# RatInABox-Lab/RatInABox

Hardware: AMD Instinct MI355X
Metric: agent-steps/sec (whole node) at 4096 agents x 1024 PlaceCells (higher is better)
Workload: dtype f32 rates / f64 motion

## Files before the change

ratinabox_amd/Neurons.py:

```python
import copy
import warnings

import numpy as np
import torch

from . import _lib, utils
from ._history import DeviceHistory, HistoryView

_Tensor = torch.Tensor

_L = _lib
LOG2E = 1.4426950408889634


def _pad4(n):
    return (int(n) + 3) // 4 * 4


class Neurons:
    default_params = {
        "n": 10,
        "name": "Neurons",
        "color": None,
        "noise_std": 0,
# ... 731 lines not shown
                self._window_stats = dict(share=self.BVC_WINDOW_SHARE, cells_need=float(keep.mean()))
                if not keep.all():
                    band = np.minimum(keep.sum(axis=1) // 24, 7)
                    order = np.lexsort((np.mod(mu_t, 2 * np.pi), band))
                    cells, vm, inv = cells[:, order], vm[order], inv[order]
                    keep = keep[order]
                    win = np.zeros(((n + 3) // 4, 2), dtype=np.int32)
                    for g in range(len(win)):
                        u = keep[np.minimum(np.arange(4 * g, 4 * g + 4), n - 1)].any(axis=0)
                        gap_len, gap_start, run = 0, 0, 0
                        for k in range(2 * K):
                            run = run + 1 if not u[k % K] else 0
                            if min(run, K) > gap_len:
                                gap_len, gap_start = min(run, K), (k - min(run, K) + 1) % K
                        first = (gap_start + gap_len) % K
                        k0 = first // 4 * 4
                        length = min(K, (first - k0 + (K - gap_len) + 3) // 4 * 4)
                        win[g] = (0, K) if length >= K else (k0, length)
                    rows_t = torch.from_numpy(order.astype(np.int32)).to(self._device)
                    win_t = torch.from_numpy(win).to(self._device)
                    self._window_stats["issued"] = float(win[:, 1].sum() * 4 / (len(win) * 4 * K))
            f32 = lambda x: torch.from_numpy(np.ascontiguousarray(x, dtype=np.float32)).to(self._device)
            s_w = walls[:, 1, :] - walls[:, 0, :]
            with np.errstate(divide="ignore"):
                rden = 1.0 / (dirs[:, None, 0] * (-s_w[None, :, 1]) + dirs[:, None, 1] * s_w[None, :, 0])
            f64 = lambda x: torch.from_numpy(np.ascontiguousarray(x, dtype=np.float64)).to(self._device)
            dirs_dev = dirs
            if os.environ.get("RIAB_EXP_NO_RAY_PAIRS"):
                dirs_dev = dirs.copy()
                dirs_dev[2, 0] += 1e-9
            return (f64(dirs_dev), f64(rden), f32(cells), f32(vm), f32(inv), rows_t, win_t)

        import os
        use_windows = os.environ.get("RIAB_NO_BVC_WINDOWS") is None
        walls = np.asarray(self.Agent.Environment.walls, dtype=np.float64).reshape(-1, 2, 2)
        dirs_t, rden_t, cells_t, vm_t, inv_t, rows_t, win_t = self._tables(
            (mu_d, sg_d, mu_t, sg_t, ang, dirs, norm, ego, walls, use_windows), build)
        if io is None:
            d = dict(kind=_L.POP_KINDS["bvc"], table=cells_t, test_dirs=dirs_t, ray_rden=rden_t, K=K, vm_table=vm_t,
                     inv_norm=inv_t, egocentric=1 if ego else 0)
            if rows_t is not None:
                d.update(cell_rows=rows_t, windows=win_t)
            return d
        env, _w = self.Agent.Environment.device_tables(self._device)
        rc = _L.lib.riab_boundary_vector_cells_windowed(env, io, _L.ptr(dirs_t), _L.ptr(rden_t), K, _L.ptr(cells_t),
                                                        _L.ptr(vm_t), _L.ptr(inv_t), n, 1 if ego else 0, None,
                                                        _L.ptr(rows_t), _L.ptr(win_t), stream)
        _L.check(rc, "riab_boundary_vector_cells")

    def _plan_scratch(self, pop):
        tiles, Kp = (self._Bp + 63) // 64, (int(pop.K) + 3) // 4 * 4
        if getattr(self, "_bvc_xch", None) is None or tuple(self._bvc_xch.shape) != (tiles, Kp, 64):
            self._bvc_xch = torch.empty((tiles, Kp, 64), dtype=torch.float32, device=self._device)
            self._bvc_xch_count = torch.zeros(tiles, dtype=torch.int32, device=self._device)
        else:
            self._bvc_xch_count.zero_()
        pop.bvc_xch, pop.bvc_xch_count = self._bvc_xch.data_ptr(), self._bvc_xch_count.data_ptr()

    def _state_op(self, d):
        from . import ops
        f = self._call(None, None)
        walls, env, periodic = self._env_op_args()
        ego = bool(f["egocentric"])
        return torch.ops.riab.boundary_vector_cells(d[0:2], d[2:4] if ego else None, walls, env, periodic, f["test_dirs"],
                                                    f["ray_rden"], f["table"], f["vm_table"], f["inv_norm"], ego,
                                                    f.get("cell_rows"), f.get("windows"), float(self.min_fr),
                                                    float(self.max_fr))


class FieldOfViewBVCs(BoundaryVectorCells):

    default_params = {
        "distance_range": [0.02, 0.4],
        "angle_range": [0, 75],
        "spatial_resolution": 0.02,
        "cell_arrangement": "diverging_manifold",
        "beta": 5,
        "color": [0.3, 0.3, 0.3, 1],
    }

    def __init__(self, Agent, params={}):
        self.params = copy.deepcopy(__class__.default_params)
        self.params.update(params)
        self.params["reference_frame"] = "egocentric"
        assert self.params["cell_arrangement"] is not None, "cell_arrangement must be set for FoV Neurons"
        self._warn_if_n_changes = "n" in params and params["n"] is not None
        super().__init__(Agent, self.params)


class ObjectVectorCells(VectorCells):

    default_params = {
        "n": 10,
        "name": "ObjectVectorCell",
        "walls_occlude": True,
        "object_tuning_type": "random",
    }

    def __init__(self, Agent, params={}):
        self.Agent = Agent
        self.params = copy.deepcopy(__class__.default_params)
        self.params.update(params)
        if not hasattr(self, "_warn_if_n_changes"):
            self._warn_if_n_changes = "n" in params and params["n"] is not None
        super().__init__(Agent, self.params)
        self.object_locations = self.Agent.Environment.objects["objects"]
        if len(self.object_locations) == 0:
            raise RuntimeError(f"Cannot initialize {self.params['name']}, as there are no objects in the environment.")
        self.tuning_types = None
        self.set_tuning_types(self.object_tuning_type)
# ... 585 lines not shown
```

ratinabox_amd/csrc/riab_bvc.hip:

```cpp
#include <type_traits>
#include "riab_device.h"
#include "riab_handover.h"
#include "riab_launch.h"

#ifndef RIAB_BVC_XCH_KB
#define RIAB_BVC_XCH_KB 1
#endif
namespace riab {

typedef float v4f __attribute__((ext_vector_type(4)));
typedef float v2f __attribute__((ext_vector_type(2)));

struct BvcArgs {
  const float* pos_x;
  const float* pos_y;
  const float* hd_x;
  const float* hd_y;
  int64_t pos_ld;
  int64_t P;
  int64_t B;
  float* rates;
  uint8_t* spikes;
  const float* u_in;
  float dt, fr_scale, fr_min;
  uint32_t k0, k1, step0, tag;
  int64_t agent_id0;
  int n, K, Kp, n_walls;
  const double* walls;
  const double* test_dirs;
  const double* ray_rden;
  const float* cells;
  const float* vm;
  const float* inv_norm;
  float* ray_out;
  const int* rows;
  const int* win;
  double e0, e1, e2, e3;
  int rect_room;
  float* xch;
  uint32_t* xch_count;
  uint32_t xch_target;
};

typedef const __attribute__((address_space(4))) double* const_f64_ptr;

template <int J>
__device__ __forceinline__ uint32_t quad_word(const u32x4& blk, int qi) {
  const uint32_t wx = (uint32_t)__builtin_amdgcn_mov_dpp((int)blk.x, J * 0x55, 0xF, 0xF, true);
  const uint32_t wy = (uint32_t)__builtin_amdgcn_mov_dpp((int)blk.y, J * 0x55, 0xF, 0xF, true);
  const uint32_t wz = (uint32_t)__builtin_amdgcn_mov_dpp((int)blk.z, J * 0x55, 0xF, 0xF, true);
  const uint32_t ww = (uint32_t)__builtin_amdgcn_mov_dpp((int)blk.w, J * 0x55, 0xF, 0xF, true);
  return qi == 0 ? wx : (qi == 1 ? wy : (qi == 2 ? wz : ww));
}

template <bool EGO>
__global__ __launch_bounds__(512) void bvc_kernel(const BvcArgs a) {
  extern __shared__ __align__(16) unsigned char smem[];
  float* s_d = reinterpret_cast<float*>(smem);
  const int tid = threadIdx.x, lane = tid & 63;
  const int wave = __builtin_amdgcn_readfirstlane(tid >> 6);
  const int nw = a.n_walls, K = a.K;
  const const_f64_ptr walls = (const_f64_ptr)(const void*)a.walls;
  const const_f64_ptr dirs = (const_f64_ptr)(const void*)a.test_dirs;
  const const_f64_ptr rden = (const_f64_ptr)(const void*)a.ray_rden;

  const int tile = (int)blockIdx.x, part = (int)blockIdx.y, nparts = (int)gridDim.y;
  const int64_t p = (int64_t)tile * 64 + lane;
  const bool live = p < a.P;
  const int64_t pc = live ? p : 0;
  const int64_t t = pc / a.B;
  const int64_t b = pc - t * a.B;
  const float pxf = a.pos_x[t * a.pos_ld + b], pyf = a.pos_y[t * a.pos_ld + b];
  const double px = pxf, py = pyf;

  bool box4 = false;
  if (a.rect_room && nw >= 4) {
    bool ok = true;
    int nh = 0, nv = 0;
    const double tol = 1e-9 * ((a.e1 - a.e0) + (a.e3 - a.e2));
    for (int w = 0; w < 4; ++w) {
      const double ax = walls[4 * w], ay = walls[4 * w + 1], bx = walls[4 * w + 2], by = walls[4 * w + 3];
      if (ay == by && ax != bx) {
        ++nh;
        ok = ok && (ay == a.e2 || ay == a.e3) && fmin(ax, bx) <= a.e0 + tol && fmax(ax, bx) >= a.e1 - tol;
      } else if (ax == bx && ay != by) {
        ++nv;
        ok = ok && (ax == a.e0 || ax == a.e1) && fmin(ay, by) <= a.e2 + tol && fmax(ay, by) >= a.e3 - tol;
      } else {
        ok = false;
      }
    }
    ok = ok && nh == 2 && nv == 2;
    const bool inside = px > a.e0 && px < a.e1 && py > a.e2 && py < a.e3;
    box4 = ok && __builtin_amdgcn_ballot_w64(live && !inside) == 0;
  }
  const int w_full = box4 ? 4 : 0;
  auto cast_rays = [&](auto KB_, const int vw, const int nvw, const bool publish) {
  constexpr int KB = decltype(KB_)::value;
  float* const xrow = publish ? a.xch + (int64_t)tile * a.Kp * 64 + lane : nullptr;
  auto put = [&](int k, float d) {
    s_d[k * 64 + lane] = d;
    if (publish) st_agent(xrow + k * 64, d);
  };
  auto stands_on_wall = [&](const double ux, const double uy, const int k) -> bool {
    for (int w = 0; w < nw; ++w) {
      const double ax = walls[4 * w], ay = walls[4 * w + 1];
      const double sx = walls[4 * w + 2] - ax, sy = walls[4 * w + 3] - ay;
      const double d0x = ax - px, d0y = ay - py;
      const double rd = rden[k * nw + w];
      const double la = (d0x * (-sy) + d0y * sx) * rd;
      const double lb = ((-d0x) * (-uy) + (-d0y) * ux) * (-rd);
      if (la == 0.0 && !(lb < 0.0) && !(lb > 1.0)) return true;
    }
    return false;
  };
  auto cast_single = [&](int count, int off) {
    for (int t0 = vw; t0 < count; t0 += nvw * KB) {
      double ux[KB], uy[KB], best[KB], fallback[KB];
      int kk[KB];
#pragma unroll
      for (int i = 0; i < KB; ++i) {
        const int t = min(t0 + nvw * i, count - 1);
        kk[i] = t == 0 ? 0 : t + off;
        ux[i] = dirs[2 * kk[i]];
        uy[i] = dirs[2 * kk[i] + 1];
        best[i] = INFINITY;
        fallback[i] = 0.0;
      }
      for (int w = 0; w < w_full; ++w) {
        const double ax = walls[4 * w], ay = walls[4 * w + 1];
        const double sx = walls[4 * w + 2] - ax, sy = walls[4 * w + 3] - ay;
        const double d0x = ax - px, d0y = ay - py;
        const double num_a = d0x * (-sy) + d0y * sx;
#pragma unroll
        for (int i = 0; i < KB; ++i) {
          const double la = num_a * rden[kk[i] * nw + w];
          if (la > 0.0 && la < best[i]) best[i] = la;
          if (w == 0) fallback[i] = la;
        }
      }
      for (int w = w_full; w < nw; ++w) {
        const double ax = walls[4 * w], ay = walls[4 * w + 1];
        const double sx = walls[4 * w + 2] - ax, sy = walls[4 * w + 3] - ay;
        const double d0x = ax - px, d0y = ay - py;
        const double num_a = d0x * (-sy) + d0y * sx;
#pragma unroll
        for (int i = 0; i < KB; ++i) {
          const double rd = rden[kk[i] * nw + w];
          const double la = num_a * rd;
          const double lb = ((-d0x) * (-uy[i]) + (-d0y) * ux[i]) * (-rd);
          const bool valid = (la > 0.0) && !(lb < 0.0) && !(lb > 1.0);
          if (valid && la < best[i]) best[i] = la;
          if (w == 0) fallback[i] = la;
        }
      }
#pragma unroll
      for (int i = 0; i < KB; ++i) {
        if (t0 + nvw * i < count) {
          const int k = kk[i];
          const bool hit = best[i] < INFINITY;
          const float d = (float)(hit ? best[i] : (stands_on_wall(ux[i], uy[i], k) ? 0.0 : fallback[i]));
          put(k, d);
          if (a.ray_out && live && (publish || part == 0)) a.ray_out[(t * K + k) * a.B + b] = d;
        }
      }
    }
  };
  const int m = K >> 1, np = K - 1 - m;
  bool paired = false;
  if ((K & 1) == 0 && np >= 8) {
    bool ok = true;
    for (int jq = 1 + lane; jq <= np; jq += 64) {
      const double e0 = a.test_dirs[2 * jq] + a.test_dirs[2 * (jq + m)];
      const double e1 = a.test_dirs[2 * jq + 1] + a.test_dirs[2 * (jq + m) + 1];
      ok = ok && fabs(e0) <= 1e-12 && fabs(e1) <= 1e-12;
    }
    paired = __builtin_amdgcn_ballot_w64(!ok) == 0;
  }
  if (paired) {
    for (int q0 = vw; q0 < np; q0 += nvw * KB) {
      double ux[KB], uy[KB], bpos[KB], bneg[KB], fallback[KB];
      int jj[KB];
#pragma unroll
      for (int i = 0; i < KB; ++i) {
        jj[i] = 1 + min(q0 + nvw * i, np - 1);
        ux[i] = dirs[2 * jj[i]];
        uy[i] = dirs[2 * jj[i] + 1];
        bpos[i] = INFINITY;
        bneg[i] = INFINITY;
        fallback[i] = 0.0;
      }
      for (int w = 0; w < w_full; ++w) {
        const double ax = walls[4 * w], ay = walls[4 * w + 1];
        const double sx = walls[4 * w + 2] - ax, sy = walls[4 * w + 3] - ay;
        const double d0x = ax - px, d0y = ay - py;
        const double num_a = d0x * (-sy) + d0y * sx;
#pragma unroll
        for (int i = 0; i < KB; ++i) {
          const double la = num_a * rden[jj[i] * nw + w];
          const double nla = -la;
          if (la > 0.0 && la < bpos[i]) bpos[i] = la;
          if (nla > 0.0 && nla < bneg[i]) bneg[i] = nla;
          if (w == 0) fallback[i] = la;
        }
      }
      for (int w = w_full; w < nw; ++w) {
        const double ax = walls[4 * w], ay = walls[4 * w + 1];
        const double sx = walls[4 * w + 2] - ax, sy = walls[4 * w + 3] - ay;
        const double d0x = ax - px, d0y = ay - py;
        const double num_a = d0x * (-sy) + d0y * sx;
#pragma unroll
        for (int i = 0; i < KB; ++i) {
          const double rd = rden[jj[i] * nw + w];
          const double la = num_a * rd;
          const double lb = ((-d0x) * (-uy[i]) + (-d0y) * ux[i]) * (-rd);
          const bool on_wall = !(lb < 0.0) && !(lb > 1.0);
          const double nla = -la;
          if (on_wall && la > 0.0 && la < bpos[i]) bpos[i] = la;
          if (on_wall && nla > 0.0 && nla < bneg[i]) bneg[i] = nla;
          if (w == 0) fallback[i] = la;
        }
      }
#pragma unroll
      for (int i = 0; i < KB; ++i) {
        if (q0 + nvw * i < np) {
          const int k = jj[i];
          const bool hit_p = bpos[i] < INFINITY, hit_n = bneg[i] < INFINITY;
          const bool on = !(hit_p && hit_n) && stands_on_wall(ux[i], uy[i], k);
          const float dp = (float)(hit_p ? bpos[i] : (on ? 0.0 : fallback[i]));
          const float dn = (float)(hit_n ? bneg[i] : (on ? 0.0 : -fallback[i]));
          put(k, dp);
          put(k + m, dn);
          if (a.ray_out && live && (publish || part == 0)) {
            a.ray_out[(t * K + k) * a.B + b] = dp;
            a.ray_out[(t * K + k + m) * a.B + b] = dn;
          }
        }
      }
    }
    cast_single(1 + (m - np), np);
  } else {
    cast_single(K, 0);
  }
  };
  const bool exchange = a.xch != nullptr && nparts > 1;
  if (!exchange) {
    cast_rays(std::integral_constant<int, 4>{}, wave, 8, false);
  } else {
    cast_rays(std::integral_constant<int, RIAB_BVC_XCH_KB>{}, wave + 8 * part, 8 * nparts, true);
    drain_stores();
    __syncthreads();
    __shared__ int s_all_here;
    if (tid == 0) {
      uint32_t* const cnt = a.xch_count + tile;
      fetch_add_agent(cnt, 1u);
      int ok = 0;
      for (int spins = 0; spins < 256; ++spins) {
        if ((int32_t)(ld_agent(cnt) - a.xch_target) >= 0) {
          ok = 1;
          break;
        }
        __builtin_amdgcn_s_sleep(8);
      }
      s_all_here = ok;
    }
    __syncthreads();
    if (s_all_here) {
      const float* const x = a.xch + (int64_t)tile * a.Kp * 64;
      for (int i = tid; i < K * 16; i += 512) {
        *reinterpret_cast<v4f*>(s_d + 4 * i) = ld_agent_v4f(x + 4 * i);
      }
    } else {
      cast_rays(std::integral_constant<int, 4>{}, wave, 8, false);
    }
  }
  for (int k = K + wave; k < a.Kp; k += 8) s_d[k * 64 + lane] = INFINITY;
  __syncthreads();

  float ch = 1.0f, sh = 0.0f;
  if (EGO) {
    const float hx = a.hd_x[t * a.pos_ld + b] + 1e-6f, hy = a.hd_y[t * a.pos_ld + b];
    const float inv = 1.0f / sqrtf(hx * hx + hy * hy);
    ch = hx * inv;
    sh = hy * inv;
  }
  const int n = a.n, Kp = a.Kp;
  const int n_groups = (n + 3) >> 2;
  for (int g = wave + 8 * part; g < n_groups; g += 8 * nparts) {
    float aa[4], nmu[4], kap[4];
    const_f32_ptr tc[4];
    const_f32_ptr ts[4];
    const const_f32_ptr cells = as_const_table(a.cells);
#pragma unroll
    for (int j = 0; j < 4; ++j) {
      const int c = min(4 * g + j, n - 1);
      nmu[j] = -cells[c];
      aa[j] = cells[n + c];
      kap[j] = cells[2 * n + c];
      tc[j] = as_const_table(a.vm + (int64_t)c * Kp);
      ts[j] = as_const_table(a.vm + ((int64_t)n + c) * Kp);
    }
    v2f acc2[4] = {{0.0f, 0.0f}, {0.0f, 0.0f}, {0.0f, 0.0f}, {0.0f, 0.0f}};
    typedef const __attribute__((address_space(4))) v4f* const_v4f_ptr;
    float d[4];
    v4f vc[4], vs[4];
    typedef const __attribute__((address_space(4))) int* const_i32_ptr;
    int k = 0, wlen = Kp;
    const int Kw = Kp;
    if (!EGO && a.win) {
      const const_i32_ptr win = (const_i32_ptr)(const void*)a.win;
      k = win[2 * g];
      wlen = win[2 * g + 1];
    }
#pragma unroll
    for (int i = 0; i < 4; ++i) d[i] = s_d[(k + i) * 64 + lane];
#pragma unroll
    for (int j = 0; j < 4; ++j) {
      vc[j] = *(const_v4f_ptr)(tc[j] + k);
      if (EGO) vs[j] = *(const_v4f_ptr)(ts[j] + k);
    }
    for (int kk = 0; kk < wlen; kk += 4) {
      const int kn = (kk + 4 < wlen) ? ((k + 4 < Kw) ? k + 4 : k + 4 - Kw) : k;
      float dn[4];
      v4f vcn[4], vsn[4];
#pragma unroll
      for (int i = 0; i < 4; ++i) dn[i] = s_d[(kn + i) * 64 + lane];
#pragma unroll
      for (int j = 0; j < 4; ++j) {
        vcn[j] = *(const_v4f_ptr)(tc[j] + kn);
        if (EGO) vsn[j] = *(const_v4f_ptr)(ts[j] + kn);
      }
#pragma unroll
      for (int j = 0; j < 4; ++j) {
#pragma unroll
        for (int i = 0; i < 4; i += 2) {
          const v2f dd = {d[i], d[i + 1]};
          const v2f tt = __builtin_elementwise_fma(dd, v2f{aa[j], aa[j]}, v2f{nmu[j], nmu[j]});
          v2f v;
          if (EGO) {
            const v2f c2 = {vc[j][i], vc[j][i + 1]}, s2 = {vs[j][i], vs[j][i + 1]};
            const v2f rot = __builtin_elementwise_fma(c2, v2f{ch, ch}, s2 * v2f{sh, sh});
// ... 9 lines not shown
      for (int i = 0; i < 4; ++i) d[i] = dn[i];
#pragma unroll
      for (int j = 0; j < 4; ++j) {
        vc[j] = vcn[j];
        if (EGO) vs[j] = vsn[j];
      }
      k = kn;
    }
    u32x4 blk = {0u, 0u, 0u, 0u};
    const int qi = lane & 3;
    if (a.spikes && !a.u_in) {
      const int ci = min(4 * g + qi, n - 1);
      const int c = a.rows ? a.rows[ci] : ci;
      const uint64_t gid = (uint64_t)(a.agent_id0 + b);
      blk = philox4x32_spikes(a.step0 + (uint32_t)t, (uint32_t)c, (uint32_t)(gid >> 2), a.tag, a.k0, a.k1);
    }
#pragma unroll
    for (int j = 0; j < 4; ++j) {
      const int ci = 4 * g + j;
      const uint32_t word = j == 0 ? quad_word<0>(blk, qi) : (j == 1 ? quad_word<1>(blk, qi) : (j == 2 ? quad_word<2>(blk, qi) : quad_word<3>(blk, qi)));
      if (ci < n && live) {
        const int c = a.rows ? a.rows[ci] : ci;
        float r = (acc2[j].x + acc2[j].y) * a.inv_norm[ci];
        r = r * a.fr_scale + a.fr_min;
        const int64_t off = (t * n + c) * a.B + b;
        if (a.P == a.B) asm volatile("global_store_dword %0, %1, off " RIAB_WT_BITS ::"v"(a.rates + off), "v"(r) : "memory");
        else a.rates[off] = r;
        if (a.spikes) {
          const float u = a.u_in ? a.u_in[off] : u01_24(word);
          a.spikes[off] = (u < a.dt * r) ? 1 : 0;
        }
      }
    }
  }
}

}

using namespace riab;

extern "C" int riab_boundary_vector_cells(const RiabEnv* env, const RiabRateIO* io, const double* test_dirs,
                                          const double* ray_rden, int32_t K, const float* cells, const float* vm_table, const float* inv_norm,
                                          int32_t n, int32_t egocentric, float* ray_out, riab_stream_t stream) {
  return riab_boundary_vector_cells_windowed(env, io, test_dirs, ray_rden, K, cells, vm_table, inv_norm, n, egocentric,
                                             ray_out, nullptr, nullptr, stream);
}

extern "C" int riab_boundary_vector_cells_windowed(const RiabEnv* env, const RiabRateIO* io, const double* test_dirs,
                                                   const double* ray_rden, int32_t K, const float* cells,
                                                   const float* vm_table, const float* inv_norm, int32_t n,
                                                   int32_t egocentric, float* ray_out, const int32_t* cell_rows,
                                                   const int32_t* windows, riab_stream_t stream) {
  return riab::launch_bvc(env, io, test_dirs, ray_rden, K, cells, vm_table, inv_norm, n, egocentric, ray_out, cell_rows, windows,
                          nullptr, nullptr, nullptr, 0, (hipStream_t)stream);
}

int riab::launch_bvc(const RiabEnv* env, const RiabRateIO* io, const double* test_dirs, const double* ray_rden, int32_t K,
                     const float* cells, const float* vm_table, const float* inv_norm, int32_t n, int32_t egocentric,
                     float* ray_out, const int32_t* cell_rows, const int32_t* windows, float* xch, uint32_t* xch_count,
                     uint32_t* xch_arrivals, int n_cus, hipStream_t stream) {
  if ((cell_rows == nullptr) != (windows == nullptr)) return RIAB_EINVAL;
  if (windows && (egocentric || K % 4 != 0)) return RIAB_EUNSUPPORTED;
  if (!env || !io || !test_dirs || !ray_rden || !cells || !vm_table || !inv_norm || n <= 0 || K <= 0) return RIAB_EINVAL;
  if (io->T <= 0 || io->B <= 0 || !io->rates || !io->pos_x || !io->pos_y) return RIAB_EINVAL;
  if (egocentric && (!io->hd_x || !io->hd_y)) return RIAB_EINVAL;
  if (env->n_walls <= 0 || !env->walls) return RIAB_EINVAL;
  if (env->n_walls > RIAB_MAX_WALLS || K > RIAB_MAX_TEST_ANGLES) return RIAB_ETOOBIG;
  if (io->u_in && !io->spikes) return RIAB_EINVAL;
  if (io->spikes && !io->u_in && (io->B % 4 != 0 || io->agent_id0 % 4 != 0)) return RIAB_EALIGN;
  BvcArgs a;
  a.pos_x = io->pos_x;
  a.pos_y = io->pos_y;
  a.hd_x = io->hd_x;
  a.hd_y = io->hd_y;
  a.pos_ld = io->pos_ld;
  a.P = io->T * io->B;
  a.B = io->B;
  a.rates = io->rates;
  a.spikes = io->spikes;
  a.u_in = io->u_in;
  a.dt = io->dt;
  a.fr_scale = io->max_fr - io->min_fr;
  a.fr_min = io->min_fr;
  a.k0 = (uint32_t)io->seed;
  a.k1 = (uint32_t)(io->seed >> 32);
  a.step0 = (uint32_t)io->step0;
  a.tag = riab::stream_tag(RIAB_TAG_SPIKES, io->pop_id);
  a.agent_id0 = io->agent_id0;
  a.n = n;
  a.K = K;
  a.Kp = (K + 3) / 4 * 4;
  a.n_walls = env->n_walls;
  a.walls = env->walls;
  a.test_dirs = test_dirs;
  a.ray_rden = ray_rden;
  a.cells = cells;
  a.vm = vm_table;
  a.inv_norm = inv_norm;
  a.ray_out = ray_out;
  a.rows = cell_rows;
  a.win = windows;
  a.e0 = env->extent[0]; a.e1 = env->extent[1]; a.e2 = env->extent[2]; a.e3 = env->extent[3];
  a.rect_room = (!env->polygon && !env->hole_mask && !env->periodic && g_options[RIAB_OPT_BVC_BOX]) ? 1 : 0;
  const size_t lds = sizeof(float) * (size_t)((K + 3) / 4 * 4) * 64;
  if (lds > 160 * 1024) return RIAB_ETOOBIG;
  const int64_t tiles = (a.P + 63) / 64;
  const int n_groups = (n + 3) / 4;
  int split = 1;
  while (split < 8 && tiles * split * 2 <= 512 && split * 2 * 8 <= n_groups) split *= 2;
  const dim3 grid((unsigned)tiles, (unsigned)split);
  if (lds > 64 * 1024) {
    const void* const fn = egocentric ? (const void*)bvc_kernel<true> : (const void*)bvc_kernel<false>;
    if (hipFuncSetAttribute(fn, hipFuncAttributeMaxDynamicSharedMemorySize, (int)lds) != hipSuccess) {
      (void)hipGetLastError();
      return RIAB_ETOOBIG;
    }
  }
  a.xch = nullptr;
  a.xch_count = nullptr;
  a.xch_target = 0u;
  hipStreamCaptureStatus cap = hipStreamCaptureStatusNone;
  const bool capturing = xch && hipStreamIsCapturing(stream, &cap) == hipSuccess && cap != hipStreamCaptureStatusNone;
  if (xch && xch_count && xch_arrivals && !capturing && split > 1 && io->T == 1 && n_cus > 0 && env->n_walls >= 8 &&
      tiles * split <= 2 * (int64_t)n_cus) {
    *xch_arrivals += (uint32_t)split;
    a.xch = xch;
    a.xch_count = xch_count;
    a.xch_target = *xch_arrivals;
  }
  hipStream_t s = (hipStream_t)stream;
  if (egocentric) hipLaunchKernelGGL(bvc_kernel<true>, grid, dim3(512), lds, s, a);
  else hipLaunchKernelGGL(bvc_kernel<false>, grid, dim3(512), lds, s, a);
  return (int)hipGetLastError();
}
```

ratinabox_amd/csrc/riab_launch.h:

```cpp
#pragma once

#include "riab_device.h"

namespace riab {

struct AgentArgs;

struct TaskRun {
  const RiabEnv* env;
  RiabTask task;
  double* task_state;
  int64_t task_B;
  double *pos_x, *pos_y;
  double* reward_out;
  uint8_t* terminal_out;
  int32_t* diag;
  int32_t auto_reset, n_select, ordered, teleport;
  int64_t agent_id0;
  uint64_t seed;
  double* ep_log;
  int64_t ep_log_cap;
  int32_t* ep_count;
  double gv_scale;
  double* world;
  uint64_t* world_met;
  int32_t *world_cand, *world_ctl;
  double t_env;
  uint64_t counter;
  float *hist_x, *hist_y;
  double *gv_x, *gv_y;
};

struct PopRows {
  const RiabEnv* env;
  const RiabPopulation* pops;
  int index;
  const float* hist;
  int64_t hist_ld;
  int64_t B;
  int32_t T;
  int64_t rate_row;
  float dt;
  uint64_t seed, step0;
  int64_t agent_id0;
  const double* state;
  double clock;
  uint32_t* xch_arrivals;
  int n_cus;
  const int64_t* cursors;
  bool write_prime;
};

int launch_population_rows(const PopRows& r, hipStream_t s, int64_t* launches);
int check_population(const RiabPopulation& q, int n_before);
inline bool population_kind_known(int kind) {
  return (kind >= RIAB_POP_PLACE && kind <= RIAB_POP_THETA_PLACE) || kind == RIAB_POP_PLANE_WAVE;
}

int launch_agent_pub(const AgentArgs& a, hipStream_t s, bool* state_published);
int launch_agent_forced(const AgentArgs& a, hipStream_t s);
int launch_agent_plain(const AgentArgs& a, hipStream_t s);
int traj_kernel_regs();
int launch_motion_task(const AgentArgs& ma, const TaskRun& t, hipStream_t s);

int launch_task_fused(const TaskRun& t, hipStream_t s);
int launch_motion_world(const AgentArgs& ma, const TaskRun& t, hipStream_t s);

int step1_supported(const RiabEnv* env, const RiabPopulation* pop, int64_t B);
int launch_step1(const AgentArgs& a, const RiabEnv* env, const Step1PopRef* refs, int n_pops, uint64_t seed, uint64_t step_after,
                 uint32_t* sync_words, uint32_t epoch, bool* walls_ready, int n_cus, hipStream_t s, bool query);
int launch_step1_task(const AgentArgs& a, const RiabEnv* env, const Step1PopRef* refs, int n_pops, uint64_t seed,
                      uint64_t step_after, uint32_t* sync_words, uint32_t epoch, bool* walls_ready, int n_cus, const TaskRun& t,
                      hipStream_t s, bool query);

int launch_bvc(const RiabEnv* env, const RiabRateIO* io, const double* test_dirs, const double* ray_rden, int32_t K,
               const float* cells, const float* vm_table, const float* inv_norm, int32_t n, int32_t egocentric,
               float* ray_out, const int32_t* cell_rows, const int32_t* windows, float* xch, uint32_t* xch_count,
               uint32_t* xch_arrivals, int n_cus, hipStream_t stream);

int td_check(const RiabTDParams* p, const RiabTDLayer* layers, int32_t n_layers);

int ovc_object_limit();

int stream_supported(const RiabEnv* env, const RiabPopulation* pop, int64_t B);
int launch_rate_stream(const RiabEnv* env, const RiabPopulation* pop, const float* hist, int64_t B, int32_t T, float dt,
                       uint64_t seed, uint64_t step0, int64_t agent_id0, uint32_t* ctrl, uint32_t spin_limit, bool stamps,
                       hipStream_t s, hipEvent_t ev_start, hipEvent_t ev_stop, bool dry_run, bool reserve,
                       uint32_t serial_rows);
int launch_stream_gate(uint32_t* ctrl, uint32_t started_target, uint32_t n_traj, uint32_t progress_target,
                       uint32_t spin_limit, bool sleep_long, uint32_t final_target, hipStream_t s);
int launch_stream_open(uint32_t* ctrl, uint32_t n_traj, uint32_t step_base, hipStream_t s);

}
```

ratinabox_amd/csrc/riab_plan.hip:

```cpp
#include <cstdlib>
#include <new>
#include <vector>

#include "riab_agent_kernel.h"
#include "riab_launch.h"

struct PlanLearner {
  int index;
  RiabTDParams p;
  float* trace[RIAB_FF_MAX_INPUTS];
  float *v_last, *dvdt, *td, *workspace;
  int64_t workspace_floats;
  int reward_kind;
  const void* reward;
  int reward_f64;
  int64_t reward_ld_n, reward_ld_b;
  int reward_index;
};

struct RiabPlan {
  RiabEnv env;
  RiabMotion motion;
  double* state;
  int64_t B;
  int64_t agent_id0;
  uint64_t seed;
  uint64_t step;
  double clock;
  uint64_t clock_step;
  const double* drift;
  const double* forced;
  int64_t forced_rows, forced_fill;
  float* hist_base;
  int64_t hist_cap, hist_fill;
  float* row_scratch;
  int32_t* diag;
  std::vector<RiabPopulation> pops;
  std::vector<int64_t> pop_fill;
  std::vector<PlanLearner> learners;
  bool has_task;
  riab::TaskRun tk;
  double dt_env;
  bool action_ready;
  uint32_t* sync_words;
  uint32_t epoch;
  bool walls_ready;
  int n_cus;
  int fused_n;
  int fused[RIAB_STEP1_MAX_POPS];
  bool fused_whole;
  int64_t fused_steps, launches;
  std::vector<uint32_t> xch_arrivals;
  std::vector<char> pre_pending;
  uint64_t pre_step;
  std::vector<int> pre_misses;
};

static int fused_agent_step(RiabPlan* p, float* row, hipStream_t s, bool need_free_row, uint32_t* mask, bool query);

static double plan_clock(RiabPlan* p) {
  for (; p->clock_step < p->step; ++p->clock_step) p->clock += p->motion.dt;
  return p->clock;
}

static uint32_t next_epoch(RiabPlan* p, bool query) {
  if (query) return 1u;
  p->epoch += 1u;
  if (p->epoch == 0u) p->epoch = 1u;
  return p->epoch;
}

static void default_compute_units(RiabPlan* p) {
  if (p->n_cus > 0) return;
  int dev = 0, n = 0;
  if (hipGetDevice(&dev) != hipSuccess || hipDeviceGetAttribute(&n, hipDeviceAttributeMultiprocessorCount, dev) != hipSuccess || n < 1) n = 1;
  p->n_cus = n;
}

static const riab::TaskRun& task_run(RiabPlan* p, float* row) {
  riab::TaskRun& t = p->tk;
  double* const act = t.gv_scale > 0.0 ? const_cast<double*>(p->drift) : nullptr;
  t.gv_x = act;
  t.gv_y = act ? act + p->B : nullptr;
  t.hist_x = row ? row + (int64_t)RIAB_H_POS_X * p->B : nullptr;
  t.hist_y = row ? row + (int64_t)RIAB_H_POS_Y * p->B : nullptr;
  return t;
}

static int fused_refs(const RiabPlan* p, riab::Step1PopRef* refs, uint32_t* mask, bool need_free_row) {
  int n = 0;
  *mask = 0u;
  for (int k = 0; k < p->fused_n; ++k) {
    const int i = p->fused[k];
    const RiabPopulation& q = p->pops[i];
    if (need_free_row && q.capacity_rows > 0 && p->pop_fill[i] >= q.capacity_rows) continue;
    const int64_t r = q.capacity_rows > 0 ? p->pop_fill[i] : 0;
    const int64_t row_elems = (int64_t)q.n * p->B;
    refs[n].pop = &q;
    refs[n].rates_row = q.rates_base + r * row_elems;
    refs[n].spikes_row = q.spikes_base ? q.spikes_base + r * row_elems : nullptr;
    *mask |= 1u << k;
    ++n;
  }
  return n;
}
// ... 336 lines not shown
  L.reward_ld_n = reward_ld_n;
  L.reward_ld_b = reward_ld_b;
  L.reward_index = reward_index;
  size_t k = 0;
  while (k < p->learners.size() && p->learners[k].index < index) ++k;
  if (k < p->learners.size() && p->learners[k].index == index) p->learners[k] = L;
  else p->learners.insert(p->learners.begin() + k, L);
  p->fused_n = -2;
  return RIAB_OK;
}

extern "C" double riab_plan_task_clock(const RiabPlan* p) { return p && p->has_task ? p->tk.t_env : 0.0; }

extern "C" int riab_plan_set_clock(RiabPlan* p, double t) {
  if (!p || !(t == t)) return RIAB_EINVAL;
  p->clock = t;
  p->clock_step = p->step;
  return RIAB_OK;
}

extern "C" double riab_plan_clock(const RiabPlan* p) { return p ? plan_clock(const_cast<RiabPlan*>(p)) : 0.0; }

extern "C" int64_t riab_plan_rows_free(const RiabPlan* p) {
  if (!p) return 0;
  int64_t free_rows = p->hist_base ? p->hist_cap - p->hist_fill : INT64_MAX;
  for (size_t i = 0; i < p->pops.size(); ++i) {
    if (p->pops[i].capacity_rows == 0) continue;
    const int64_t f = p->pops[i].capacity_rows - p->pop_fill[i];
    free_rows = f < free_rows ? f : free_rows;
  }
  return free_rows;
}

extern "C" uint64_t riab_plan_step_index(const RiabPlan* p) { return p ? p->step : 0; }

int riab::launch_population_rows(const PopRows& r, hipStream_t s, int64_t* launches) {
  const RiabEnv* env = r.env;
  const RiabPopulation& q = r.pops[r.index];
  const int64_t B = r.B;
  RiabRateIO io = q.io;
  hist_rows_io(&io, r.hist, B, r.hist_ld);
  io.T = r.T;
  io.rates = q.rates_base + r.rate_row * q.n * B;
  io.spikes = q.spikes_base ? q.spikes_base + r.rate_row * q.n * B : nullptr;
  io.u_in = nullptr;
  io.dt = r.dt;
  io.seed = r.seed;
  io.step0 = r.step0;
  io.agent_id0 = r.agent_id0;
  const bool noisy = q.noise_state != nullptr;
  uint8_t* const spikes = io.spikes;
  if (noisy) io.spikes = nullptr;
  int rc = RIAB_EUNSUPPORTED;
  switch (q.kind) {
    case RIAB_POP_PLACE: rc = riab_place_cells(env, &io, q.table, q.n, q.description, q.geometry, q.top_hat_width, s); break;
    case RIAB_POP_GRID: rc = riab_grid_cells(&io, q.table, q.n, q.description, q.f0, s); break;
    case RIAB_POP_HDC: rc = riab_head_direction_cells(&io, q.table, q.n, s); break;
    case RIAB_POP_PLANE_WAVE: rc = riab_plane_wave_neurons(&io, q.table, q.n, s); break;
    case RIAB_POP_VELOCITY:
      if (!r.state) break;
      rc = riab_velocity_cells(&io, q.table, q.n, q.one_sigma_speed, r.state + RIAB_S_VEL_X * B, r.state + RIAB_S_VEL_Y * B, s);
      break;
    case RIAB_POP_THETA_PLACE:
      if (!r.state) break;
      rc = riab_phase_precessing_place_cells(env, &io, q.table, q.n, q.description, q.geometry, q.top_hat_width, q.kappa,
                                             q.theta_freq * fmod(r.clock, 1.0 / q.theta_freq), r.state + RIAB_S_VEL_X * B,
                                             r.state + RIAB_S_VEL_Y * B, s);
      break;
    case RIAB_POP_SPEED:
      io.hd_x = r.hist + RIAB_H_VEL_X * B;
      io.hd_y = r.hist + RIAB_H_VEL_Y * B;
      rc = riab_speed_cell(&io, q.one_sigma_speed, s);
      break;
    case RIAB_POP_RANDOM_SPATIAL:
      rc = riab_random_spatial_neurons(env, &io, q.table, q.n_anchors, q.targets, q.n, q.geometry, s);
      break;
    case RIAB_POP_BVC: {
      const bool xch = r.xch_arrivals != nullptr;
      rc = launch_bvc(env, &io, q.test_dirs, q.ray_rden, q.K, q.table, q.vm_table, q.inv_norm, q.n, q.egocentric, nullptr,
                      q.cell_rows, q.windows, xch ? q.bvc_xch : nullptr, xch ? q.bvc_xch_count : nullptr, r.xch_arrivals,
                      xch ? r.n_cus : 0, s);
      break;
    }
    case RIAB_POP_OVC:
      rc = riab_object_vector_cells(env, &io, q.objects, q.object_types, q.n_objects, q.table, q.n, q.walls_occlude,
                                    q.egocentric, s);
      break;
    case RIAB_POP_FF: {
      RiabFFInput in[RIAB_FF_MAX_INPUTS];
      for (int l = 0; l < q.n_inputs; ++l) {
        const int j = q.input_index[l];
        const RiabPopulation& src = r.pops[j];
        const int64_t row_j = !r.cursors ? r.rate_row : (src.capacity_rows > 0 ? r.cursors[j] - 1 : 0);
        in[l].rates = src.rates_base + row_j * src.n * B;
        in[l].wt = q.input_wt[l];
        in[l].n_in = src.n;
      }
      rc = riab_feedforward(in, q.n_inputs, q.bias, q.n, r.T, B, q.activation, q.act_params, io.rates,
                            r.write_prime ? q.rates_prime : nullptr, s);
      if (rc == RIAB_OK && io.spikes) rc = riab_spikes(&io, q.n, s);
      break;
    }
  }
  if (rc) return rc;
  if (launches) *launches += (q.kind == RIAB_POP_FF && io.spikes) ? 2 : 1;
  if (noisy) {
    if (launches) *launches += spikes ? 2 : 1;
    rc = riab_neuron_noise(q.noise_state, io.rates, nullptr, q.n, B, r.T, q.noise_theta_dt, q.noise_sigma_dt, r.seed, r.step0,
                           q.io.pop_id, r.agent_id0, s);
    if (rc) return rc;
    if (spikes) {
      io.spikes = spikes;
      rc = riab_spikes(&io, q.n, s);
    }
  }
  return rc;
}

static int launch_population(RiabPlan* p, size_t i, const float* row, hipStream_t s) {
  riab::PopRows r = {};
  r.env = &p->env;
  r.pops = p->pops.data();
  r.index = (int)i;
  r.hist = row;
  r.hist_ld = p->B;
  r.B = p->B;
  r.T = 1;
  r.rate_row = p->pop_fill[i];
  r.dt = (float)p->motion.dt;
  r.seed = p->seed;
  r.step0 = p->step;
  r.agent_id0 = p->agent_id0;
  r.state = p->state;
  if (p->pops[i].kind == RIAB_POP_THETA_PLACE) r.clock = plan_clock(p);
  if (p->pops[i].kind == RIAB_POP_BVC) {
    default_compute_units(p);
    if (p->xch_arrivals.size() < p->pops.size()) p->xch_arrivals.resize(p->pops.size(), 0u);
    r.xch_arrivals = &p->xch_arrivals[i];
    r.n_cus = p->n_cus;
  }
  r.cursors = p->pop_fill.data();
  r.write_prime = true;
  return riab::launch_population_rows(r, s, &p->launches);
}

static void count_missed_rows(RiabPlan* p) {
  for (size_t i = 0; i < p->pre_pending.size(); ++i) {
    if (!p->pre_pending[i]) continue;
    p->pre_pending[i] = 0;
    if (++p->pre_misses[i] == 2) p->fused_n = -2;
  }
}

static void advance_cursors(RiabPlan* p, bool task) {
  p->step += 1;
  if (p->hist_base) p->hist_fill += 1;
  if (task) {
    p->tk.t_env += p->dt_env;
    if (p->tk.auto_reset) p->tk.counter += 1;
  }
}

extern "C" int riab_plan_step_agent(RiabPlan* p, riab_stream_t stream) {
  if (!p || p->has_task) return RIAB_EINVAL;
  if (!p->learners.empty()) return RIAB_EUNSUPPORTED;
  if (p->hist_base && p->hist_fill >= p->hist_cap) return RIAB_EFULL;
  const double* forced = nullptr;
  if (p->forced) {
    if (p->forced_fill >= p->forced_rows) return RIAB_EFULL;
    forced = p->forced + p->forced_fill * 2 * p->B;
  }
  float* row = p->hist_base ? p->hist_base + p->hist_fill * (int64_t)RIAB_HIST_ROWS * p->B : p->row_scratch;
  count_missed_rows(p);
  if (plan_fused(p) > 0) {
    uint32_t mask = 0u;
    const int rc = fused_agent_step(p, row, (hipStream_t)stream, true, &mask, false);
    if (rc == RIAB_OK) {
      advance_cursors(p, false);
      for (int k = 0; k < p->fused_n; ++k)
        if (mask & (1u << k)) p->pre_pending[p->fused[k]] = 1;
      p->pre_step = p->step;
      return RIAB_OK;
    }
    if (rc != RIAB_EUNSUPPORTED) return rc;
  }
  const int rc = riab_agent_step(&p->env, &p->motion, p->state, p->B, p->agent_id0, p->drift, nullptr, nullptr, forced, nullptr,
                                 p->seed, p->step, 1, row, p->diag, (hipStream_t)stream);
  if (rc) return rc;
  p->launches += 1;
  if (forced) p->forced_fill += 1;
  advance_cursors(p, false);
  return RIAB_OK;
}
// ... 230 lines not shown
```

Measured before the change: 1.425 billion.

## Split BVC ray casting into a separate kernel instead of inter-block spin exchange

Replaces the in-kernel cross-block exchange, where split blocks published ray distances and spin-waited on an atomic arrival counter, with a dedicated ray-casting kernel. That kernel fills the exchange buffer across a 2-D grid, and the main BVC kernel then just loads it into LDS. Ray casting is factored into reusable device functions, and the per-cell group loop now deals groups across parts in an interleaved rank order. This removes the atomic counter, its zeroing, and the spin/fallback path, at the cost of an extra kernel launch and a global round-trip for the ray distances. The workload here is place cells, so BVC paths are likely not exercised.

```diff
diff --git a/ratinabox_amd/Neurons.py b/ratinabox_amd/Neurons.py
--- a/ratinabox_amd/Neurons.py
+++ b/ratinabox_amd/Neurons.py
@@ -807,10 +807,7 @@
         tiles, Kp = (self._Bp + 63) // 64, (int(pop.K) + 3) // 4 * 4
         if getattr(self, "_bvc_xch", None) is None or tuple(self._bvc_xch.shape) != (tiles, Kp, 64):
             self._bvc_xch = torch.empty((tiles, Kp, 64), dtype=torch.float32, device=self._device)
-            self._bvc_xch_count = torch.zeros(tiles, dtype=torch.int32, device=self._device)
-        else:
-            self._bvc_xch_count.zero_()
-        pop.bvc_xch, pop.bvc_xch_count = self._bvc_xch.data_ptr(), self._bvc_xch_count.data_ptr()
+        pop.bvc_xch, pop.bvc_xch_count = self._bvc_xch.data_ptr(), None
 
     def _state_op(self, d):
         from . import ops
diff --git a/ratinabox_amd/csrc/riab_bvc.hip b/ratinabox_amd/csrc/riab_bvc.hip
--- a/ratinabox_amd/csrc/riab_bvc.hip
+++ b/ratinabox_amd/csrc/riab_bvc.hip
@@ -1,11 +1,7 @@
-#include <type_traits>
 #include "riab_device.h"
 #include "riab_handover.h"
 #include "riab_launch.h"
 
-#ifndef RIAB_BVC_XCH_KB
-#define RIAB_BVC_XCH_KB 1
-#endif
 namespace riab {
 
 typedef float v4f __attribute__((ext_vector_type(4)));
@@ -38,69 +34,81 @@
   double e0, e1, e2, e3;
   int rect_room;
   float* xch;
-  uint32_t* xch_count;
-  uint32_t xch_target;
+  int rays_ready;
 };
 
 typedef const __attribute__((address_space(4))) double* const_f64_ptr;
 
-template <int J>
-__device__ __forceinline__ uint32_t quad_word(const u32x4& blk, int qi) {
-  const uint32_t wx = (uint32_t)__builtin_amdgcn_mov_dpp((int)blk.x, J * 0x55, 0xF, 0xF, true);
-  const uint32_t wy = (uint32_t)__builtin_amdgcn_mov_dpp((int)blk.y, J * 0x55, 0xF, 0xF, true);
-  const uint32_t wz = (uint32_t)__builtin_amdgcn_mov_dpp((int)blk.z, J * 0x55, 0xF, 0xF, true);
-  const uint32_t ww = (uint32_t)__builtin_amdgcn_mov_dpp((int)blk.w, J * 0x55, 0xF, 0xF, true);
-  return qi == 0 ? wx : (qi == 1 ? wy : (qi == 2 ? wz : ww));
-}
-
-template <bool EGO>
-__global__ __launch_bounds__(512) void bvc_kernel(const BvcArgs a) {
-  extern __shared__ __align__(16) unsigned char smem[];
-  float* s_d = reinterpret_cast<float*>(smem);
-  const int tid = threadIdx.x, lane = tid & 63;
-  const int wave = __builtin_amdgcn_readfirstlane(tid >> 6);
-  const int nw = a.n_walls, K = a.K;
+
+struct RayLane {
+  int lane;
+  bool live;
+  int64_t t, b;
+  double px, py;
+};
+
+__device__ __forceinline__ RayLane ray_lane(const BvcArgs& a, int tile, int lane) {
+  RayLane r;
+  r.lane = lane;
+  const int64_t p = (int64_t)tile * 64 + lane;
+  r.live = p < a.P;
+  const int64_t pc = r.live ? p : 0;
+  r.t = pc / a.B;
+  r.b = pc - r.t * a.B;
+  r.px = a.pos_x[r.t * a.pos_ld + r.b];
+  r.py = a.pos_y[r.t * a.pos_ld + r.b];
+  return r;
+}
+
+__device__ __forceinline__ bool box_fast_path(const BvcArgs& a, const RayLane& r) {
+  const const_f64_ptr walls = (const_f64_ptr)(const void*)a.walls;
+  if (!a.rect_room || a.n_walls < 4) return false;
+  bool ok = true;
+  int nh = 0, nv = 0;
+  const double tol = 1e-9 * ((a.e1 - a.e0) + (a.e3 - a.e2));
+  for (int w = 0; w < 4; ++w) {
+    const double ax = walls[4 * w], ay = walls[4 * w + 1], bx = walls[4 * w + 2], by = walls[4 * w + 3];
+    if (ay == by && ax != bx) {
+      ++nh;
+      ok = ok && (ay == a.e2 || ay == a.e3) && fmin(ax, bx) <= a.e0 + tol && fmax(ax, bx) >= a.e1 - tol;
+    } else if (ax == bx && ay != by) {
+      ++nv;
+      ok = ok && (ax == a.e0 || ax == a.e1) && fmin(ay, by) <= a.e2 + tol && fmax(ay, by) >= a.e3 - tol;
+    } else {
+      ok = false;
+    }
+  }
+  ok = ok && nh == 2 && nv == 2;
+  const bool inside = r.px > a.e0 && r.px < a.e1 && r.py > a.e2 && r.py < a.e3;
+  return ok && __builtin_amdgcn_ballot_w64(r.live && !inside) == 0;
+}
+
+__device__ __forceinline__ bool dirs_paired(const BvcArgs& a, int lane) {
+  const int K = a.K, m = K >> 1, np = K - 1 - m;
+  if ((K & 1) != 0 || np < 8) return false;
+  bool ok = true;
+  for (int jq = 1 + lane; jq <= np; jq += 64) {
+    const double e0 = a.test_dirs[2 * jq] + a.test_dirs[2 * (jq + m)];
+    const double e1 = a.test_dirs[2 * jq + 1] + a.test_dirs[2 * (jq + m) + 1];
+    ok = ok && fabs(e0) <= 1e-12 && fabs(e1) <= 1e-12;
+  }
+  return __builtin_amdgcn_ballot_w64(!ok) == 0;
+}
+
+template <int KB>
+__device__ __forceinline__ void cast_rays(const BvcArgs& a, const RayLane& r, const bool box4, const bool paired, const int vw,
+                                          const int vw1, const int nvw, float* const s_d, float* const xrow,
+                                          const bool to_ray_out) {
+  const int nw = a.n_walls, K = a.K, lane = r.lane;
   const const_f64_ptr walls = (const_f64_ptr)(const void*)a.walls;
   const const_f64_ptr dirs = (const_f64_ptr)(const void*)a.test_dirs;
   const const_f64_ptr rden = (const_f64_ptr)(const void*)a.ray_rden;
-
-  const int tile = (int)blockIdx.x, part = (int)blockIdx.y, nparts = (int)gridDim.y;
-  const int64_t p = (int64_t)tile * 64 + lane;
-  const bool live = p < a.P;
-  const int64_t pc = live ? p : 0;
-  const int64_t t = pc / a.B;
-  const int64_t b = pc - t * a.B;
-  const float pxf = a.pos_x[t * a.pos_ld + b], pyf = a.pos_y[t * a.pos_ld + b];
-  const double px = pxf, py = pyf;
-
-  bool box4 = false;
-  if (a.rect_room && nw >= 4) {
-    bool ok = true;
-    int nh = 0, nv = 0;
-    const double tol = 1e-9 * ((a.e1 - a.e0) + (a.e3 - a.e2));
-    for (int w = 0; w < 4; ++w) {
-      const double ax = walls[4 * w], ay = walls[4 * w + 1], bx = walls[4 * w + 2], by = walls[4 * w + 3];
-      if (ay == by && ax != bx) {
-        ++nh;
-        ok = ok && (ay == a.e2 || ay == a.e3) && fmin(ax, bx) <= a.e0 + tol && fmax(ax, bx) >= a.e1 - tol;
-      } else if (ax == bx && ay != by) {
-        ++nv;
-        ok = ok && (ax == a.e0 || ax == a.e1) && fmin(ay, by) <= a.e2 + tol && fmax(ay, by) >= a.e3 - tol;
-      } else {
-        ok = false;
-      }
-    }
-    ok = ok && nh == 2 && nv == 2;
-    const bool inside = px > a.e0 && px < a.e1 && py > a.e2 && py < a.e3;
-    box4 = ok && __builtin_amdgcn_ballot_w64(live && !inside) == 0;
-  }
+  const double px = r.px, py = r.py;
+  const int64_t t = r.t, b = r.b;
   const int w_full = box4 ? 4 : 0;
-  auto cast_rays = [&](auto KB_, const int vw, const int nvw, const bool publish) {
-  constexpr int KB = decltype(KB_)::value;
-  float* const xrow = publish ? a.xch + (int64_t)tile * a.Kp * 64 + lane : nullptr;
   auto put = [&](int k, float d) {
-    s_d[k * 64 + lane] = d;
-    if (publish) st_agent(xrow + k * 64, d);
+    if (s_d) s_d[k * 64 + lane] = d;
+    if (xrow) st_agent(xrow + k * 64, d);
   };
   auto stands_on_wall = [&](const double ux, const double uy, const int k) -> bool {
     for (int w = 0; w < nw; ++w) {
@@ -114,8 +122,8 @@
     }
     return false;
   };
-  auto cast_single = [&](int count, int off) {
-    for (int t0 = vw; t0 < count; t0 += nvw * KB) {
+  auto cast_single = [&](int count, int off, int v) {
+    for (int t0 = v; t0 < count; t0 += nvw * KB) {
       double ux[KB], uy[KB], best[KB], fallback[KB];
       int kk[KB];
 #pragma unroll
@@ -161,22 +169,12 @@
           const bool hit = best[i] < INFINITY;
           const float d = (float)(hit ? best[i] : (stands_on_wall(ux[i], uy[i], k) ? 0.0 : fallback[i]));
           put(k, d);
-          if (a.ray_out && live && (publish || part == 0)) a.ray_out[(t * K + k) * a.B + b] = d;
+          if (to_ray_out) a.ray_out[(t * K + k) * a.B + b] = d;
         }
       }
     }
   };
   const int m = K >> 1, np = K - 1 - m;
-  bool paired = false;
-  if ((K & 1) == 0 && np >= 8) {
-    bool ok = true;
-    for (int jq = 1 + lane; jq <= np; jq += 64) {
-      const double e0 = a.test_dirs[2 * jq] + a.test_dirs[2 * (jq + m)];
-      const double e1 = a.test_dirs[2 * jq + 1] + a.test_dirs[2 * (jq + m) + 1];
-      ok = ok && fabs(e0) <= 1e-12 && fabs(e1) <= 1e-12;
-    }
-    paired = __builtin_amdgcn_ballot_w64(!ok) == 0;
-  }
   if (paired) {
     for (int q0 = vw; q0 < np; q0 += nvw * KB) {
       double ux[KB], uy[KB], bpos[KB], bneg[KB], fallback[KB];
@@ -231,48 +229,68 @@
           const float dn = (float)(hit_n ? bneg[i] : (on ? 0.0 : -fallback[i]));
           put(k, dp);
           put(k + m, dn);
-          if (a.ray_out && live && (publish || part == 0)) {
+          if (to_ray_out) {
             a.ray_out[(t * K + k) * a.B + b] = dp;
             a.ray_out[(t * K + k + m) * a.B + b] = dn;
           }
         }
       }
     }
-    cast_single(1 + (m - np), np);
+    cast_single(1 + (m - np), np, vw1);
   } else {
-    cast_single(K, 0);
-  }
-  };
-  const bool exchange = a.xch != nullptr && nparts > 1;
-  if (!exchange) {
-    cast_rays(std::integral_constant<int, 4>{}, wave, 8, false);
+    cast_single(K, 0, vw);
+  }
+}
+
+#ifndef RIAB_BVC_RAYS_KB
+#define RIAB_BVC_RAYS_KB 1
+#endif
+#define RIAB_BVC_PAIR_MIN_WALLS 8
+
+__global__ __launch_bounds__(512) void bvc_rays_kernel(const BvcArgs a) {
+  const int tid = threadIdx.x, lane = tid & 63;
+  const int wave = __builtin_amdgcn_readfirstlane(tid >> 6);
+  const int tile = (int)blockIdx.x, vw = wave + 8 * (int)blockIdx.y, nvw = 8 * (int)gridDim.y;
+  const RayLane r = ray_lane(a, tile, lane);
+  const bool box4 = box_fast_path(a, r);
+  const bool paired = dirs_paired(a, lane);
+  const int np = a.K - 1 - (a.K >> 1);
+  const int vw1 = (vw + nvw - np % nvw) % nvw;
+  float* const xrow = a.xch + (int64_t)tile * a.Kp * 64 + lane;
+  cast_rays<RIAB_BVC_RAYS_KB>(a, r, box4, paired, vw, vw1, nvw, nullptr, xrow, a.ray_out && r.live);
+  if (vw == nvw - 1) {
+    for (int k = a.K; k < a.Kp; ++k) st_agent(xrow + k * 64, INFINITY);
+  }
+}
+
+template <int J>
+__device__ __forceinline__ uint32_t quad_word(const u32x4& blk, int qi) {
+  const uint32_t wx = (uint32_t)__builtin_amdgcn_mov_dpp((int)blk.x, J * 0x55, 0xF, 0xF, true);
+  const uint32_t wy = (uint32_t)__builtin_amdgcn_mov_dpp((int)blk.y, J * 0x55, 0xF, 0xF, true);
+  const uint32_t wz = (uint32_t)__builtin_amdgcn_mov_dpp((int)blk.z, J * 0x55, 0xF, 0xF, true);
+  const uint32_t ww = (uint32_t)__builtin_amdgcn_mov_dpp((int)blk.w, J * 0x55, 0xF, 0xF, true);
+  return qi == 0 ? wx : (qi == 1 ? wy : (qi == 2 ? wz : ww));
+}
+
+template <bool EGO>
+__global__ __launch_bounds__(512) void bvc_kernel(const BvcArgs a) {
+  extern __shared__ __align__(16) unsigned char smem[];
+  float* s_d = reinterpret_cast<float*>(smem);
+  const int tid = threadIdx.x, lane = tid & 63;
+  const int wave = __builtin_amdgcn_readfirstlane(tid >> 6);
+  const int K = a.K;
+
+  const int tile = (int)blockIdx.x, part = (int)blockIdx.y, nparts = (int)gridDim.y;
+  const RayLane r = ray_lane(a, tile, lane);
+  const bool live = r.live;
+  const int64_t t = r.t, b = r.b;
+
+  if (a.rays_ready) {
+    const float* const x = a.xch + (int64_t)tile * a.Kp * 64;
+    for (int i = tid; i < K * 16; i += 512) *reinterpret_cast<v4f*>(s_d + 4 * i) = *reinterpret_cast<const v4f*>(x + 4 * i);
   } else {
-    cast_rays(std::integral_constant<int, RIAB_BVC_XCH_KB>{}, wave + 8 * part, 8 * nparts, true);
-    drain_stores();
-    __syncthreads();
-    __shared__ int s_all_here;
-    if (tid == 0) {
-      uint32_t* const cnt = a.xch_count + tile;
-      fetch_add_agent(cnt, 1u);
-      int ok = 0;
-      for (int spins = 0; spins < 256; ++spins) {
-        if ((int32_t)(ld_agent(cnt) - a.xch_target) >= 0) {
-          ok = 1;
-          break;
-        }
-        __builtin_amdgcn_s_sleep(8);
-      }
-      s_all_here = ok;
-    }
-    __syncthreads();
-    if (s_all_here) {
-      const float* const x = a.xch + (int64_t)tile * a.Kp * 64;
-      for (int i = tid; i < K * 16; i += 512) {
-        *reinterpret_cast<v4f*>(s_d + 4 * i) = ld_agent_v4f(x + 4 * i);
-      }
-    } else {
-      cast_rays(std::integral_constant<int, 4>{}, wave, 8, false);
-    }
+    cast_rays<4>(a, r, box_fast_path(a, r), dirs_paired(a, lane), wave, wave, 8, s_d, nullptr,
+                 a.ray_out && live && part == 0);
   }
   for (int k = K + wave; k < a.Kp; k += 8) s_d[k * 64 + lane] = INFINITY;
   __syncthreads();
@@ -286,7 +304,9 @@
   }
   const int n = a.n, Kp = a.Kp;
   const int n_groups = (n + 3) >> 2;
-  for (int g = wave + 8 * part; g < n_groups; g += 8 * nparts) {
+  const bool deal = nparts > 1;
+  const int rank = wave < 4 ? 2 * wave : 15 - 2 * wave;
+  for (int g = deal ? part + nparts * rank : wave + 8 * part; g < n_groups; g += 8 * nparts) {
     float aa[4], nmu[4], kap[4];
     const_f32_ptr tc[4];
     const_f32_ptr ts[4];
@@ -402,13 +422,13 @@
                                                    int32_t egocentric, float* ray_out, const int32_t* cell_rows,
                                                    const int32_t* windows, riab_stream_t stream) {
   return riab::launch_bvc(env, io, test_dirs, ray_rden, K, cells, vm_table, inv_norm, n, egocentric, ray_out, cell_rows, windows,
-                          nullptr, nullptr, nullptr, 0, (hipStream_t)stream);
+                          nullptr, nullptr, (hipStream_t)stream);
 }
 
 int riab::launch_bvc(const RiabEnv* env, const RiabRateIO* io, const double* test_dirs, const double* ray_rden, int32_t K,
                      const float* cells, const float* vm_table, const float* inv_norm, int32_t n, int32_t egocentric,
-                     float* ray_out, const int32_t* cell_rows, const int32_t* windows, float* xch, uint32_t* xch_count,
-                     uint32_t* xch_arrivals, int n_cus, hipStream_t stream) {
+                     float* ray_out, const int32_t* cell_rows, const int32_t* windows, float* xch, int* n_launched,
+                     hipStream_t stream) {
   if ((cell_rows == nullptr) != (windows == nullptr)) return RIAB_EINVAL;
   if (windows && (egocentric || K % 4 != 0)) return RIAB_EUNSUPPORTED;
   if (!env || !io || !test_dirs || !ray_rden || !cells || !vm_table || !inv_norm || n <= 0 || K <= 0) return RIAB_EINVAL;
@@ -466,19 +486,23 @@
       return RIAB_ETOOBIG;
     }
   }
+  hipStream_t s = (hipStream_t)stream;
   a.xch = nullptr;
-  a.xch_count = nullptr;
-  a.xch_target = 0u;
-  hipStreamCaptureStatus cap = hipStreamCaptureStatusNone;
-  const bool capturing = xch && hipStreamIsCapturing(stream, &cap) == hipSuccess && cap != hipStreamCaptureStatusNone;
-  if (xch && xch_count && xch_arrivals && !capturing && split > 1 && io->T == 1 && n_cus > 0 && env->n_walls >= 8 &&
-      tiles * split <= 2 * (int64_t)n_cus) {
-    *xch_arrivals += (uint32_t)split;
+  a.rays_ready = 0;
+  if (n_launched) *n_launched = 1;
+  if (xch && split > 1 && io->T == 1 && env->n_walls >= RIAB_BVC_PAIR_MIN_WALLS) {
+    const int m = K >> 1, np = K - 1 - m;
+    const int items = ((K & 1) == 0 && np >= 8) ? np + 1 + (m - np) : K;
+    int gy = (items + 7) / 8;
+    const int gy_max = (int)(1024 / tiles) > 1 ? (int)(1024 / tiles) : 1;
+    gy = gy < gy_max ? gy : gy_max;
     a.xch = xch;
-    a.xch_count = xch_count;
-    a.xch_target = *xch_arrivals;
-  }
-  hipStream_t s = (hipStream_t)stream;
+    hipLaunchKernelGGL(bvc_rays_kernel, dim3((unsigned)tiles, (unsigned)gy), dim3(512), 0, s, a);
+    const int rc = (int)hipGetLastError();
+    if (rc) return rc;
+    a.rays_ready = 1;
+    if (n_launched) *n_launched = 2;
+  }
   if (egocentric) hipLaunchKernelGGL(bvc_kernel<true>, grid, dim3(512), lds, s, a);
   else hipLaunchKernelGGL(bvc_kernel<false>, grid, dim3(512), lds, s, a);
   return (int)hipGetLastError();
diff --git a/ratinabox_amd/csrc/riab_launch.h b/ratinabox_amd/csrc/riab_launch.h
--- a/ratinabox_amd/csrc/riab_launch.h
+++ b/ratinabox_amd/csrc/riab_launch.h
@@ -45,8 +45,7 @@
   int64_t agent_id0;
   const double* state;
   double clock;
-  uint32_t* xch_arrivals;
-  int n_cus;
+  bool bvc_ray_kernel;
   const int64_t* cursors;
   bool write_prime;
 };
@@ -75,8 +74,8 @@
 
 int launch_bvc(const RiabEnv* env, const RiabRateIO* io, const double* test_dirs, const double* ray_rden, int32_t K,
                const float* cells, const float* vm_table, const float* inv_norm, int32_t n, int32_t egocentric,
-               float* ray_out, const int32_t* cell_rows, const int32_t* windows, float* xch, uint32_t* xch_count,
-               uint32_t* xch_arrivals, int n_cus, hipStream_t stream);
+               float* ray_out, const int32_t* cell_rows, const int32_t* windows, float* xch, int* n_launched,
+               hipStream_t stream);
 
 int td_check(const RiabTDParams* p, const RiabTDLayer* layers, int32_t n_layers);
 
diff --git a/ratinabox_amd/csrc/riab_plan.hip b/ratinabox_amd/csrc/riab_plan.hip
--- a/ratinabox_amd/csrc/riab_plan.hip
+++ b/ratinabox_amd/csrc/riab_plan.hip
@@ -50,7 +50,6 @@
   int fused[RIAB_STEP1_MAX_POPS];
   bool fused_whole;
   int64_t fused_steps, launches;
-  std::vector<uint32_t> xch_arrivals;
   std::vector<char> pre_pending;
   uint64_t pre_step;
   std::vector<int> pre_misses;
@@ -493,6 +492,7 @@
   uint8_t* const spikes = io.spikes;
   if (noisy) io.spikes = nullptr;
   int rc = RIAB_EUNSUPPORTED;
+  int n_kernels = 1;
   switch (q.kind) {
     case RIAB_POP_PLACE: rc = riab_place_cells(env, &io, q.table, q.n, q.description, q.geometry, q.top_hat_width, s); break;
     case RIAB_POP_GRID: rc = riab_grid_cells(&io, q.table, q.n, q.description, q.f0, s); break;
@@ -517,10 +517,8 @@
       rc = riab_random_spatial_neurons(env, &io, q.table, q.n_anchors, q.targets, q.n, q.geometry, s);
       break;
     case RIAB_POP_BVC: {
-      const bool xch = r.xch_arrivals != nullptr;
       rc = launch_bvc(env, &io, q.test_dirs, q.ray_rden, q.K, q.table, q.vm_table, q.inv_norm, q.n, q.egocentric, nullptr,
-                      q.cell_rows, q.windows, xch ? q.bvc_xch : nullptr, xch ? q.bvc_xch_count : nullptr, r.xch_arrivals,
-                      xch ? r.n_cus : 0, s);
+                      q.cell_rows, q.windows, r.bvc_ray_kernel ? q.bvc_xch : nullptr, &n_kernels, s);
       break;
     }
     case RIAB_POP_OVC:
@@ -544,7 +542,7 @@
     }
   }
   if (rc) return rc;
-  if (launches) *launches += (q.kind == RIAB_POP_FF && io.spikes) ? 2 : 1;
+  if (launches) *launches += (q.kind == RIAB_POP_FF && io.spikes) ? 2 : n_kernels;
   if (noisy) {
     if (launches) *launches += spikes ? 2 : 1;
     rc = riab_neuron_noise(q.noise_state, io.rates, nullptr, q.n, B, r.T, q.noise_theta_dt, q.noise_sigma_dt, r.seed, r.step0,
@@ -574,12 +572,7 @@
   r.agent_id0 = p->agent_id0;
   r.state = p->state;
   if (p->pops[i].kind == RIAB_POP_THETA_PLACE) r.clock = plan_clock(p);
-  if (p->pops[i].kind == RIAB_POP_BVC) {
-    default_compute_units(p);
-    if (p->xch_arrivals.size() < p->pops.size()) p->xch_arrivals.resize(p->pops.size(), 0u);
-    r.xch_arrivals = &p->xch_arrivals[i];
-    r.n_cus = p->n_cus;
-  }
+  r.bvc_ray_kernel = true;
   r.cursors = p->pop_fill.data();
   r.write_prime = true;
   return riab::launch_population_rows(r, s, &p->launches);
```

Result: slower. 1.404 billion (-1.5%).
